# yizuo417/RollingDepth

Measured on AMD Instinct MI355X. Metric: depth frames/sec at 768px snip_len=3, 1-step denoise; 1/2/4/8 MI355X, higher is better.
Workload: dtype f16; 1 GPU; fast preset: 100-frame 768x768 video, dilations [1, 25] (cap_dilation=True), snippet_len 3, 1-step DDIM, aligner 2000 it, refine 0; SD2-shaped UNet+VAE random-init; preset=fast, frames=100, res=768, parallelism=snippet-dp1

## Files before the change

### include/rdmi.h

```cpp
#ifndef RDMI_H
#define RDMI_H

#include <stddef.h>

#ifdef __cplusplus
extern "C" {
#endif

#define RDMI_OK 0
#define RDMI_E_ARG 1001
#define RDMI_E_ALIGN 1002
#define RDMI_E_UNSUPPORTED 1003

#define RDMI_F16 0
#define RDMI_F32 1
#define RDMI_U8 2
#define RDMI_F32_X3 3
#define RDMI_F32_X6 4

#define RDMI_RESIZE_NEAREST 0
#define RDMI_RESIZE_BILINEAR 1
#define RDMI_RESIZE_BICUBIC 2

#define RDMI_EPI_NONE 0
// ... 105 lines not shown
  float* workspace;
  int start_step[8];
} rdmi_aligner_args;
long rdmi_aligner_workspace(const rdmi_aligner_args* a);
int rdmi_aligner_optimize(const rdmi_aligner_args* a, void* stream);
int rdmi_aligner_prepare(const void* x, int x_f32, int n, int w, int H, int W, int border,
                         int factor, const float* shift, float* out, void* stream);
int rdmi_aligner_merge(int n_dil, const void* const* xf, int x_f32, const float* const* s,
                       const float* const* t, const int* n, const int* stride, const int* w, int seq_len,
                       long HW, const float* shift, float* out, void* stream);
int rdmi_aligner_merge_strided(int n_dil, const void* const* xf, int x_f32, const float* const* s,
                               const float* const* t, const int* n, const int* stride, const int* start_step,
                               const int* w, int seq_len, long HW, const float* shift, float* out, void* stream);

int rdmi_aligner_merge_partial_window(int n_dil, const void* const* xf, int x_f32, const float* const* s,
                                      const float* const* t, const int* n, const int* stride, const int* k0,
                                      const int* nloc, const int* w, int f0, int nf, long HW, const float* shift,
                                      double* sum_out, void* stream);
int rdmi_aligner_merge_finish_pieces(int n_dil, const int* n, const int* stride, const int* w, int f0, int nf, long HW,
                                     int npieces, const int* piece_f0, const int* piece_nf, const double* recv,
                                     float* out, void* stream);
int rdmi_aligner_merge_partial_window_strided(int n_dil, const void* const* xf, int x_f32, const float* const* s,
                                              const float* const* t, const int* n, const int* stride,
                                              const int* start_step, const int* k0, const int* nloc, const int* w,
                                              int seq_len, int f0, int nf, long HW, const float* shift,
                                              double* sum_out, void* stream);
int rdmi_aligner_merge_finish_pieces_strided(int n_dil, const int* n, const int* stride, const int* start_step,
                                             const int* w, int seq_len, int f0, int nf, long HW, int npieces,
                                             const int* piece_f0, const int* piece_nf, const double* recv,
                                             float* out, void* stream);

int rdmi_attention_d512(const void* q, const void* k, const void* vt, void* o, int B, int Sq, int Sk, int Skp,
                        long q_ld, long k_ld, long vt_ld, long o_ld, long q_bs, long k_bs, long vt_bs, long o_bs,
                        float scale, int* flags, void* stream);

size_t rdmi_resize_workspace(int N, int C, int H, int W, int Ho, int Wo);
int rdmi_resize(const void* x, int x_dtype, long sn, long sc, long sy, long sx, int N, int C, int H, int W, int Ho,
                int Wo, int mode, int normalize, float* y, void* workspace, void* stream);

#ifdef __cplusplus
}
#endif
#endif
```

### rollingdepth_amd/_native.py

```python
from __future__ import annotations

import ctypes as C
import os

_LIB_PATH = os.environ.get("RDMI_LIB") or os.path.join(os.path.dirname(os.path.abspath(__file__)), "_lib", "librdmi.so")

vp = C.c_void_p
i32 = C.c_int
i64 = C.c_long
f32 = C.c_float


class GemmArgs(C.Structure):
    _fields_ = [
        ("A", vp), ("lda", i64), ("strideA", i64),
        ("W", vp), ("ldw", i64), ("strideW", i64),
        ("C", vp), ("ldc", i64), ("strideC", i64), ("c_f32", i32),
        ("bias", vp),
        ("residual", vp), ("ldr", i64), ("strideR", i64),
        ("rowbias", vp), ("rows_per_group", i32), ("rowbias_ld", i64),
        ("alpha", f32),
        ("M", i32), ("N", i32), ("K", i32), ("batch", i32),
        ("epilogue", i32),
        ("gn_part", vp), ("gn_ld", i64),
# ... 31 lines not shown
    ]


_SIGS = {
    "rdmi_last_error": (C.c_char_p, []),
    "rdmi_version": (i32, []),
    "rdmi_gemm": (i32, [C.POINTER(GemmArgs), vp]),
    "rdmi_conv2d": (i32, [C.POINTER(ConvArgs), vp]),
    "rdmi_conv2d_in_gn_supported": (i32, [C.POINTER(ConvArgs)]),
    "rdmi_groupnorm_workspace": (i64, [i32, i32]),
    "rdmi_groupnorm_stats": (i32, [vp, i32, i32, i64, i32, i32, f32, vp, vp, vp]),
    "rdmi_groupnorm_stats_partials": (i32, [vp, i64, i32, i64, i32, i32, f32, vp, vp]),
    "rdmi_groupnorm_apply": (i32, [vp, vp, i32, i32, i64, i32, i32, vp, vp, vp, i32, vp]),
    "rdmi_conv3x3_to1_gn_workspace": (i64, [i32, i32, i32]),
    "rdmi_conv3x3_to1_gn": (i32, [vp, i32, i32, i32, i32, i32, i32, vp, vp, vp, i32, vp, f32, vp, i32, vp, vp]),
    "rdmi_layernorm": (i32, [vp, vp, i32, i64, i32, vp, vp, f32, vp]),
    "rdmi_attention_fwd": (i32, [vp, vp, vp, vp, i32, i32, i32, i32, i32, i64, i64, i64, i64, i64, i64, i64, i64,
                                 f32, i32, vp]),
    "rdmi_attention_smallkv": (i32, [vp, vp, vp, vp, i32, i32, i32, i32, i32, i64, i64, i64, i64, i64, f32, i32, vp]),
    "rdmi_cross_attn_pair": (i32, [vp, vp, i64, i32, i32, vp, vp, f32, vp, vp, vp, vp]),
    "rdmi_softmax_rows": (i32, [vp, vp, i64, i64, i64, f32, i32, vp]),
    "rdmi_nchw_to_nhwc": (i32, [vp, i32, vp, i32, i32, i32, i32, i32, i32, f32, i64, i64, vp]),
    "rdmi_nhwc_to_nchw_f32": (i32, [vp, i32, i64, vp, i32, i32, i32, i32, f32, f32, vp]),
    "rdmi_concat_channels": (i32, [vp, i32, vp, i32, vp, i64, i32, vp]),
    "rdmi_resize_nearest": (i32, [vp, i32, i32, i32, i32, vp, i32, i32, i32, vp]),
    "rdmi_transpose": (i32, [vp, vp, i32, i64, i64, i64, i64, i32, vp]),
    "rdmi_gather_unet_input": (i32, [vp, i64, vp, i64, i32, vp, i32, i64, vp, i32, vp]),
    "rdmi_ddim_combine": (i32, [vp, i64, vp, i64, vp, i64, i64, i32, i32, f32, f32, f32, i64, i32, vp]),
    "rdmi_snippet_average": (i32, [vp, i32, i32, i32, i32, i64, i32, i32, vp, i32, vp]),
    "rdmi_snippet_accumulate": (i32, [vp, i32, i32, i32, i32, i32, i32, i64, i32, i32, vp, vp]),
    "rdmi_snippet_finish": (i32, [vp, i32, i32, i32, i32, i64, i32, i32, vp, i32, vp]),
    "rdmi_colorize": (i32, [vp, i32, i64, vp, vp, i32, vp, vp, vp]),
    "rdmi_resize_workspace": (C.c_size_t, [i32, i32, i32, i32, i32, i32]),
    "rdmi_attention_d512": (i32, [vp, vp, vp, vp, i32, i32, i32, i32] + [i64] * 8 + [C.c_float, vp, vp]),
    "rdmi_resize": (i32, [vp, i32, i64, i64, i64, i64, i32, i32, i32, i32, i32, i32, i32, i32, vp, vp, vp]),
    "rdmi_minmax": (i32, [vp, i32, i64, vp, vp, vp]),
    "rdmi_renormalize_f32": (i32, [vp, i64, vp, vp]),
    "rdmi_aligner_workspace": (i64, [C.POINTER(AlignerArgs)]),
    "rdmi_aligner_optimize": (i32, [C.POINTER(AlignerArgs), vp]),
    "rdmi_aligner_prepare": (i32, [vp, i32, i32, i32, i32, i32, i32, i32, vp, vp, vp]),
    "rdmi_aligner_merge": (i32, [i32, C.POINTER(vp), i32, C.POINTER(vp), C.POINTER(vp), C.POINTER(i32),
                                 C.POINTER(i32), C.POINTER(i32), i32, i64, vp, vp, vp]),
    "rdmi_aligner_merge_strided": (i32, [i32, C.POINTER(vp), i32, C.POINTER(vp), C.POINTER(vp), C.POINTER(i32),
                                         C.POINTER(i32), C.POINTER(i32), C.POINTER(i32), i32, i64, vp, vp, vp]),
    "rdmi_groupnorm_affine": (i32, [vp, vp, vp, i32, i32, i32, vp, vp]),
    "rdmi_aligner_merge_partial_window": (i32, [i32, C.POINTER(vp), i32, C.POINTER(vp), C.POINTER(vp),
                                                C.POINTER(i32), C.POINTER(i32), C.POINTER(i32), C.POINTER(i32),
                                                C.POINTER(i32), i32, i32, i64, vp, vp, vp]),
    "rdmi_aligner_merge_finish_pieces": (i32, [i32, C.POINTER(i32), C.POINTER(i32), C.POINTER(i32), i32, i32, i64,
                                               i32, C.POINTER(i32), C.POINTER(i32), vp, vp, vp]),
    "rdmi_aligner_merge_partial_window_strided": (i32, [i32, C.POINTER(vp), i32, C.POINTER(vp), C.POINTER(vp),
                                                        C.POINTER(i32), C.POINTER(i32), C.POINTER(i32),
                                                        C.POINTER(i32), C.POINTER(i32), C.POINTER(i32), i32, i32, i32,
                                                        i64, vp, vp, vp]),
    "rdmi_aligner_merge_finish_pieces_strided": (i32, [i32, C.POINTER(i32), C.POINTER(i32), C.POINTER(i32),
                                                       C.POINTER(i32), i32, i32, i32, i64, i32, C.POINTER(i32),
                                                       C.POINTER(i32), vp, vp, vp]),
}

RDMI_F16, RDMI_F32, RDMI_U8, RDMI_F32_X3, RDMI_F32_X6 = 0, 1, 2, 3, 4
RDMI_RESIZE_NEAREST, RDMI_RESIZE_BILINEAR, RDMI_RESIZE_BICUBIC = 0, 1, 2

EXPORTED = tuple(_SIGS)


def _load():
    if not os.path.exists(_LIB_PATH):
# ... 23 lines not shown
```

### rollingdepth_amd/csrc/attention_d512.hip

```cpp
#include "common.h"

namespace {

constexpr int D5 = 512;
constexpr int NW5 = 8;
constexpr int QB5 = 16 * NW5;
constexpr int KT5 = 32;
constexpr int KTILE = KT5 * D5;
constexpr int STAGE = 2 * KTILE;
constexpr int PPW = 32 / NW5;

__device__ __forceinline__ int kswz(int k) { return (k & 3) | (((k >> 3) & 3) << 2); }
__device__ __forceinline__ int vswz(int d) { return ((d >> 3) & 1) * 3; }

struct Attn512P {
  const f16* q; const f16* k; const f16* vt; f16* o;
  int Sq, Sk, Skp;
  long q_ld, k_ld, vt_ld, o_ld, q_bs, k_bs, vt_bs, o_bs;
  float c;
  int* flags;
};

__global__ __launch_bounds__(64 * NW5, 1) void attn_fwd_d512(Attn512P p) {
  __shared__ __attribute__((aligned(16))) f16 lds5[2 * STAGE];
// ... 102 lines not shown
#pragma unroll
          for (int db = 0; db < 32; ++db) o[db] *= alpha;
        }
        mt = mnew;
      }
      rs = 0.f;
#pragma unroll
      for (int e = 0; e < 8; ++e) {
        pv[e] = __builtin_amdgcn_exp2f(fmaf(s[e >> 2][e & 3], p.c, -mt));
        rs += pv[e];
      }
      rs += __shfl_xor(rs, 16, 64);
      rs += __shfl_xor(rs, 32, 64);
    }
    l += rs;
    f16x8 pf;
#pragma unroll
    for (int e = 0; e < 8; ++e) pf[e] = (f16)pv[e];
#pragma unroll
    for (int db = 0; db < 32; ++db) {
      const f16x8 vf = *(const f16x8*)LDS_PTR(f16, (uintptr_t)(st + vaddr + db * 1024));
      o[db] = __builtin_amdgcn_mfma_f32_16x16x32_f16(vf, pf, o[db], 0, 0, 0);
    }
  }
  if (q < p.Sq) {
    const float inv = 1.f / l;
    f16* O = p.o + (long)b * p.o_bs + (long)q * p.o_ld;
#pragma unroll
    for (int db = 0; db < 32; ++db) {
      f16x4 w;
#pragma unroll
      for (int r = 0; r < 4; ++r) w[r] = (f16)(o[db][r] * inv);
      *(f16x4*)(O + 16 * db + 4 * hq) = w;
    }
  }
}


__device__ __forceinline__ int kswz32(int k) { return k & 15; }
__device__ __forceinline__ int vswz32(int d) { return (d >> 2) & 3; }

template <int N>
__device__ __forceinline__ void w4_sched() {
#pragma unroll
  for (int i = 0; i < N; ++i) {
    __builtin_amdgcn_sched_group_barrier(0x100, 1, 0);
    __builtin_amdgcn_sched_group_barrier(0x008, 1, 0);
  }
}

__global__ __launch_bounds__(256, 1) void attn_fwd_d512_w4(Attn512P p) {
  __shared__ __attribute__((aligned(16))) f16 lds5[2 * STAGE];
  const int tid = threadIdx.x;
  const int lane = tid & 63;
  const int wid = tid >> 6;
  const int hh = lane >> 5;
  const int j32 = lane & 31;
  const int qblk = blockIdx.x, b = blockIdx.y;
  const int q = qblk * 128 + wid * 32 + j32;

  const f16* Q = p.q + (long)b * p.q_bs;
  const __amdgpu_buffer_rsrc_t rk = __builtin_amdgcn_make_buffer_rsrc(
      (void*)(p.k + (long)b * p.k_bs), (short)0, (int)(((long)(p.Sk - 1) * p.k_ld + D5) * 2), 0x00020000);
  const __amdgpu_buffer_rsrc_t rv = __builtin_amdgcn_make_buffer_rsrc(
      (void*)(p.vt + (long)b * p.vt_bs), (short)0, (int)(((long)(D5 - 1) * p.vt_ld + p.Skp) * 2), 0x00020000);

// ... 83 lines not shown
#pragma unroll
    for (int db = 0; db < 16; ++db)
#pragma unroll
      for (int s2 = 0; s2 < 2; ++s2) {
        const f16x8 vf = *(const f16x8*)LDS_PTR(f16, (uintptr_t)(st + vaddr[s2] + db * 2048));
        o[db] = __builtin_amdgcn_mfma_f32_32x32x16_f16(vf, pf[s2], o[db], 0, 0, 0);
      }
    w4_sched<32>();
  }
  int* badw = (int*)lds5;
  __syncthreads();
  if (lane == 0) badw[wid] = bad;
  __syncthreads();
  if (tid == 0) p.flags[b * gridDim.x + qblk] = badw[0] | badw[1] | badw[2] | badw[3];
  if (q < p.Sq && !bad) {
    const float inv = 1.f / l;
    f16* O = p.o + (long)b * p.o_bs + (long)q * p.o_ld;
#pragma unroll
    for (int db = 0; db < 16; ++db)
#pragma unroll
      for (int jx = 0; jx < 4; ++jx) {
        f16x4 w;
#pragma unroll
        for (int r = 0; r < 4; ++r) w[r] = (f16)(o[db][4 * jx + r] * inv);
        *(f16x4*)(O + 32 * db + 8 * jx + 4 * hh) = w;
      }
  }
}

}

extern "C" int rdmi_attention_d512(const void* q, const void* k, const void* vt, void* o, int B, int Sq, int Sk, int Skp,
                                   long q_ld, long k_ld, long vt_ld, long o_ld, long q_bs, long k_bs, long vt_bs,
                                   long o_bs, float scale, int* flags, void* stream) {
  RDMI_REQUIRE(q && k && vt && o, RDMI_E_ARG, "attention_d512: null pointer");
  RDMI_REQUIRE(B > 0 && Sq > 0 && Sk > 0 && Skp >= Sk && Skp % 32 == 0 && vt_ld >= Skp, RDMI_E_ARG,
               "attention_d512: bad sizes (Skp %% 32 == 0, Skp >= Sk, vt_ld >= Skp)");
  RDMI_REQUIRE(q_ld % 8 == 0 && k_ld % 8 == 0 && vt_ld % 8 == 0 && o_ld % 4 == 0 &&
                   (((uintptr_t)q | (uintptr_t)k | (uintptr_t)vt) & 15) == 0 && ((uintptr_t)o & 7) == 0,
               RDMI_E_ALIGN, "attention_d512: strides / pointers not aligned");
  RDMI_REQUIRE((long)(Sk - 1) * k_ld + D5 < (1L << 30) && (long)(D5 - 1) * vt_ld + Skp < (1L << 30), RDMI_E_ARG,
               "attention_d512: K / Vᵀ exceed the 2 GiB buffer range");
  Attn512P p{(const f16*)q, (const f16*)k, (const f16*)vt, (f16*)o, Sq, Sk, Skp, q_ld, k_ld, vt_ld, o_ld,
             q_bs, k_bs, vt_bs, o_bs, scale * 1.4426950408889634f, flags};
  const dim3 grid(rdmi::div_up(Sq, QB5), B);
  if (flags) {
    hipLaunchKernelGGL(attn_fwd_d512_w4, grid, dim3(256), 0, (hipStream_t)stream, p);
    if (int e = rdmi::check_launch("attention_d512 (32-query pass)")) return e;
  }
  hipLaunchKernelGGL(attn_fwd_d512, grid, dim3(64 * NW5), 0, (hipStream_t)stream, p);
  return rdmi::check_launch("attention_d512");
}
```

### rollingdepth_amd/kernels.py

```python
from __future__ import annotations

import ctypes as C
import math
import os
from typing import Optional, Sequence, Tuple

import torch

from . import _native as _N
from ._native import check, lib

F16 = torch.float16
F32 = torch.float32


def _stream() -> int:
    return torch.cuda.current_stream().cuda_stream


_PROF = None


def profile_start():
    global _PROF
# ... 615 lines not shown
    if out.numel() != rows * p_ld or not out.is_contiguous() or p_ld < cols:
        raise ValueError("softmax_rows: out must be a contiguous [..., >= cols] tensor")
    check(lib.rdmi_softmax_rows(s.data_ptr(), out.data_ptr(), rows, cols, p_ld, scale, _dtype_code(out), _stream()),
          "rdmi_softmax_rows")
    return out


def attention_1head(q: torch.Tensor, k: torch.Tensor, v: torch.Tensor, scale: float) -> torch.Tensor:
    B, Sq, D = q.shape
    Sk = k.shape[1]
    if D == 512 and q.dtype == F16 and os.environ.get("RDMI_VAE_FLASH", "1") != "0":
        return attention_d512(q, k, v, scale)
    s = gemm(q, k, D, out_f32=True)
    Sp = (Sk + 7) // 8 * 8
    p = softmax_rows(s, scale, out=torch.empty((B, Sq, Sp), dtype=q.dtype, device=q.device))
    del s
    vt = torch.zeros((B, D, Sp), dtype=q.dtype, device=q.device) if Sp != Sk else None
    vt = transpose(v, out=vt)
    return gemm(p, vt, Sp)


def attention_d512(q: torch.Tensor, k: torch.Tensor, v: torch.Tensor, scale: float) -> torch.Tensor:
    B, Sq, D = q.shape
    Sk = k.shape[1]
    if D != 512 or q.dtype != F16 or k.dtype != F16 or v.dtype != F16:
        raise ValueError("attention_d512: f16 q / k / v with head dim 512")
    Skp = (Sk + 31) // 32 * 32
    vt = torch.zeros((B, D, Skp), dtype=F16, device=q.device) if Skp != Sk else None
    vt = transpose(v, out=vt)
    o = torch.empty((B, Sq, D), dtype=F16, device=q.device)
    flags = None
    if os.environ.get("RDMI_D512_W4", "0") == "1":
        flags = torch.empty((B * ((Sq + 127) // 128),), dtype=torch.int32, device=q.device)
    with _Timed("attention_d512", 4.0 * B * Sq * Sk * D, f"attn512 B={B} S={Sq}", 2 * B * D * (2 * Sq + 2 * Sk)):
        check(lib.rdmi_attention_d512(q.data_ptr(), k.data_ptr(), vt.data_ptr(), o.data_ptr(), B, Sq, Sk, Skp,
                                      q.stride(1), k.stride(1), vt.stride(1), o.stride(1), q.stride(0), k.stride(0),
                                      vt.stride(0), o.stride(0), float(scale),
                                      flags.data_ptr() if flags is not None else None, _stream()),
              "rdmi_attention_d512")
    return o


def transpose(src: torch.Tensor, out: Optional[torch.Tensor] = None) -> torch.Tensor:
    _need_act(src, "transpose.src")
    B, R, Cc = src.shape
    out = torch.empty((B, Cc, R), dtype=src.dtype, device=src.device) if out is None else out
    for t, rows, nm in ((src, R, "src"), (out, Cc, "out")):
        if t.stride(2) != 1 or (B > 1 and t.stride(0) != rows * t.stride(1)):
            raise ValueError(f"transpose: {nm} strides {t.stride()} (unit column stride, batch stride = rows · row "
                             f"stride expected)")
    check(lib.rdmi_transpose(src.data_ptr(), out.data_ptr(), B, R, Cc, src.stride(1), out.stride(1), _dtype_code(src),
                             _stream()), "rdmi_transpose")
    return out


def nchw_to_nhwc(x: torch.Tensor, cpad: int, scale: float = 1.0, dtype=F16) -> torch.Tensor:
    if not x.is_cuda or x.dtype not in (F16, F32):
        raise TypeError("nchw_to_nhwc: device f16/f32 tensor expected")
    B, Cc, H, W = x.shape
    if x.stride(3) != 1 or x.stride(2) != W:
        x = x.contiguous()
    out = torch.empty((B, H, W, cpad), dtype=dtype, device=x.device)
    check(lib.rdmi_nchw_to_nhwc(x.data_ptr(), int(x.dtype == F32), out.data_ptr(), _dtype_code(out), B, Cc, H, W, cpad,
                                scale, x.stride(0), x.stride(1), _stream()), "rdmi_nchw_to_nhwc")
    return out


def nhwc_to_nchw_f32(x: torch.Tensor, c: int, scale: float = 1.0, shift: float = 0.0) -> torch.Tensor:
    _need_act(x, "nhwc_to_nchw.x")
    B, H, W, Cl = x.shape
# ... 285 lines not shown
```

### rollingdepth_amd/csrc/conv_occ2.hip

```cpp
#include "gemm_kernels.h"

namespace rdmi_gk {

template <int MODE>
static void occ2_mode_launch(bool gn, bool pipe, dim3 g, hipStream_t s, const GemmP& p) {
  if (gn && pipe)
    hipLaunchKernelGGL((conv_halo_occ2_kernel<MODE, true, true>), g, dim3(256), 0, s, p);
  else if (gn)
    hipLaunchKernelGGL((conv_halo_occ2_kernel<MODE, true, false>), g, dim3(256), 0, s, p);
  else if (pipe)
    hipLaunchKernelGGL((conv_halo_occ2_kernel<MODE, false, true>), g, dim3(256), 0, s, p);
  else
    hipLaunchKernelGGL((conv_halo_occ2_kernel<MODE, false, false>), g, dim3(256), 0, s, p);
}

void launch_conv_occ2(int mode, bool gn, bool pipe, dim3 g, hipStream_t s, const GemmP& p) {
  if (mode == 3) {
    if (pipe)
      hipLaunchKernelGGL((conv_halo_occ2_kernel<3, false, true>), g, dim3(256), 0, s, p);
    else
      hipLaunchKernelGGL((conv_halo_occ2_kernel<3, false, false>), g, dim3(256), 0, s, p);
  } else if (mode == 2)
    occ2_mode_launch<2>(gn, pipe, g, s, p);
  else
    occ2_mode_launch<1>(gn, pipe, g, s, p);
}

void launch_conv_h32(bool gn, dim3 g, hipStream_t s, const GemmP& p) {
  if (gn)
    hipLaunchKernelGGL((conv_halo32_kernel<true>), g, dim3(256), 0, s, p);
  else
    hipLaunchKernelGGL((conv_halo32_kernel<false>), g, dim3(256), 0, s, p);
}

void launch_gemm_occ2(int bn, dim3 g, hipStream_t s, const GemmP& p) {
  if (bn == 160 && !p.geglu)
    hipLaunchKernelGGL((gemm_occ2_kernel<0, 160>), g, dim3(256), 0, s, p);
  else
    hipLaunchKernelGGL((gemm_occ2_kernel<0, 128>), g, dim3(256), 0, s, p);
}

}
```

### rollingdepth_amd/csrc/gemm.hip

```cpp
#include "gemm_kernels.h"

#include <stdlib.h>

namespace {

using namespace rdmi_gk;


int occ2_mode() {
  const char* e = getenv("RDMI_GEMM_OCC2");
  return e ? atoi(e) : 1;
}

int pp_mode() {
  const char* e = getenv("RDMI_GEMM_PP");
  return e ? atoi(e) : 1;
}

double tile_cost(long tiles, int bm, int bn, double eff) {
  return (double)((tiles + 255) / 256) * bm * bn / eff;
}

template <int MODE, int WM, int RN>
void launch_pp(const GemmP& p, int batch, hipStream_t s) {
// ... 206 lines not shown
    const char* xp = getenv("RDMI_XFORM_PRIO");
    p.xprio = !(xp && xp[0] == '0');
    const char* ep = getenv("RDMI_EPI_PRIO");
    p.eprio = ep && ep[0] == '1';
    const char* cp = getenv("RDMI_CPERM");
    p.cperm = (!cp || cp[0] != '0') && p.vec && ((uintptr_t)p.C & 15) == 0 && p.ldc % 8 == 0 &&
              (!p.R || (((uintptr_t)p.R & 15) == 0 && p.ldr % 8 == 0));
    p.gmr = a->in_mean_rstd; p.ggam = a->in_gamma; p.gbet = a->in_beta; p.gG = a->in_groups; p.gsilu = a->in_silu;
    p.gaff = a->in_mean_rstd ? a->in_affine : nullptr;
    RDMI_REQUIRE(!p.gaff || ((uintptr_t)p.gaff & 15) == 0, RDMI_E_ALIGN, "conv2d: in_affine not 16-byte aligned");
    hipStream_t st = (hipStream_t)stream;
    const unsigned patches = (unsigned)((a->Ho / 16) * (a->Wo / 16) * a->B);
    const bool gn = p.gmr != nullptr;
    if (a->upsample && a->w_up2 && !gn && a->Ho % 32 == 0 && a->Wo % 32 == 0 && al16(a->w_up2)) {
      p.Wt = (const f16*)a->w_up2; p.ldw = 7L * a->Cin; p.K = p.Kvalid = 7 * a->Cin;
      p.w_bytes = (unsigned)(4L * a->Cout * p.ldw * 2);
      launch_conv_occ2(3, false, p.conv_pipe != 0, dim3((a->Cout + 127) / 128, patches, 1), st, p);
    } else if (a->Cout % 256 == 0 && !p.gaff && !(hmode == 3 && (!gn || a->Cin <= 256))) {
      dim3 g(a->Cout / 256, patches, 1);
      const bool ph2 = hmode != 1 || gn;
      if (a->upsample) {
        launch_conv_halo(2, ph2 ? 2 : 4, 4, ph2 && gn, g, st, p);
      } else {
        launch_conv_halo(1, ph2 ? 2 : 4, 4, ph2 && gn, g, st, p);
      }
    } else if (a->Cout == 128 && !p.gaff && (hmode == 4 || (gn && a->Cin > 256))) {
      dim3 g(1, patches, 1);
      launch_conv_halo(a->upsample ? 2 : 1, 1, 2, gn, g, st, p);
    } else if (h32_ok(a, p, gn)) {
      dim3 g(a->Cout / 128, (unsigned)((a->Ho / 8) * (a->Wo / 32) * a->B), 1);
      launch_conv_h32(gn, g, st, p);
    } else {
      dim3 g((a->Cout + 127) / 128, patches, 1);
      launch_conv_occ2(a->upsample ? 2 : 1, gn, p.conv_pipe != 0, g, st, p);
    }
    return rdmi::check_launch("conv2d halo");
  }
  if (dense && conv1x1_ok(p) && launch_conv1x1(p, a->Cin, a->Cout, (hipStream_t)stream))
    return rdmi::check_launch("conv2d 1x1");
  return launch(p, 1, (hipStream_t)stream, false, dense ? 0 : (a->upsample ? 2 : 1));
}
```

### rollingdepth_amd/csrc/gemm_kernels.h

```cpp
#pragma once
#include "common.h"

#include <utility>

namespace rdmi_gk {

constexpr int BK = 64;

struct GemmP {
  const f16* A; long lda, sA;
  const f16* Wt; long ldw, sW;
  void* C; long ldc, sC; int c_f32;
  const float* bias;
  const f16* R; long ldr, sR;
  const float* rowbias; int rpg; long rb_ld;
  float alpha;
  int M, N, K, Kvalid;
  int geglu, silu, vec;
  unsigned a_bytes, w_bytes;
  int IH, IW, Cin, Ho, Wo, kh, kw, stride, pt, pl, up, cin_vecs;
  int cmaj;
  float* gnp; long gn_ld;
  int group_m;
  const float* gmr; const float* ggam; const float* gbet; int gG, gsilu;
// ... 1122 lines not shown
      asm volatile("" ::: "memory");
      __builtin_amdgcn_s_barrier();
      asm volatile("" ::: "memory");
      seg(5);
    }
  }
  if (grp == 0) __builtin_amdgcn_s_barrier();
  wait_vmcnt<0>();
  seg(5);

  store_tile<RM, RN, 64, true>(p, acc, PatchRows{b, p.Ho, p.Wo, y0, x0, wm * RM, fr}, n0 + wn * 64, 0, fr, fq, p.cperm);
  if constexpr (STAMP) {
    wait_vmcnt<0>();
    seg(6);
    st_acc[7] = st_prev - st_start;
    if (lane == 0) {
      unsigned long long* o = p.stamps + (((long)blockIdx.y * gridDim.x + blockIdx.x) * 8 + wid) * 8;
      for (int i = 0; i < 8; ++i) o[i] = st_acc[i];
    }
  }
}

template <int RN, int PD, int NS, int BPRE, int ST>
__device__ __forceinline__ void occ2_sched_one() {
  constexpr int nr = (ST == BPRE ? RN : 0) + (ST + PD < NS ? 1 : 0);
  if constexpr (nr > 0) __builtin_amdgcn_sched_group_barrier(0x100, nr, 0);
  __builtin_amdgcn_sched_group_barrier(0x008, RN, 0);
}
template <int RN, int PD, int NS, int BPRE, int... S>
__device__ __forceinline__ void occ2_sched(std::integer_sequence<int, S...>) {
  (occ2_sched_one<RN, PD, NS, BPRE, S>(), ...);
}

template <int MODE, bool GN, bool PIPE, int STAMP = 0>
__global__ __launch_bounds__(256, 2) void conv_halo_occ2_kernel(GemmP p) {
  unsigned long long st_acc[6] = {}, st_prev = 0, st_start = 0;
  auto seg = [&](int i) __attribute__((always_inline)) {
    if constexpr (STAMP) {
      const unsigned long long t = gk_stamp();
      st_acc[i] += t - st_prev;
      st_prev = t;
    }
  };
  if constexpr (STAMP) st_start = st_prev = gk_stamp();
  constexpr int BN = 128, BKP = 64, RM = 8, RN = 4;
  constexpr int HWD = 18, HPIX = HWD * HWD;
  constexpr int HPC = 41;
  constexpr int HPW = 11;
  constexpr int HALO = HPC * 8 * BKP;
  constexpr int BSLOT = BN * BKP;
  constexpr int NB = 4;
  constexpr int GNT = GN ? 256 : 0;
  constexpr int PREF = 4 * 2 * 64 * 2;
  __shared__ __attribute__((aligned(16))) f16 lds[HALO + 2 * BSLOT + 4 * GNT + PREF];
  float* const gnt = (float*)(lds + HALO + 2 * BSLOT);

  const int tid = threadIdx.x;
  const int lane = tid & 63;
  const int wid = tid >> 6;
  const int wm = wid >> 1, wn = wid & 1;
  const int wids = __builtin_amdgcn_readfirstlane(wid);
  const int nbx = gridDim.x;
  int mt_, nt_;
  if (p.group_m < 0 && nbx > 1 && 8 % nbx == 0 && gridDim.y % (8 / nbx) == 0) {
    const int bid = blockIdx.y * nbx + blockIdx.x, xcd = bid & 7;
    nt_ = xcd % nbx;
    mt_ = (bid >> 3) * (8 / nbx) + xcd / nbx;
  } else {
    const int logical = xcd_remap(blockIdx.y * nbx + blockIdx.x, nbx * gridDim.y);
    tile_mn(logical, nbx, gridDim.y, p.group_m, mt_, nt_);
  }
  const int n0 = nt_ * BN;
  constexpr int NT = MODE == 3 ? 7 : 9;
  const int pxn = p.Wo >> (MODE == 3 ? 5 : 4), pyn = p.Ho >> (MODE == 3 ? 5 : 4);
  const int px = mt_ % pxn;
  const int py = (mt_ / pxn) % pyn;
  const int phs = MODE == 3 ? (mt_ / (pxn * pyn)) & 3 : 0;
  const int b = mt_ / (pxn * pyn * (MODE == 3 ? 4 : 1));
  const int pa = phs >> 1, pc = phs & 1;
  const int y0 = py * 16, x0 = px * 16;
  const __amdgpu_buffer_rsrc_t ra_ =
      __builtin_amdgcn_make_buffer_rsrc((void*)p.A, (short)0, (int)p.a_bytes, 0x00020000);
  const __amdgpu_buffer_rsrc_t rw_ =
      __builtin_amdgcn_make_buffer_rsrc((void*)p.Wt, (short)0, (int)p.w_bytes, 0x00020000);

  const int lrow = lane >> 3;
  const int chunk = (lane & 7) ^ lrow;
  const int Hl = p.IH << (MODE == 2 ? 1 : 0), Wl = p.IW << (MODE == 2 ? 1 : 0);
  unsigned hvo[HPW];
#pragma unroll
  for (int e = 0; e < HPW; ++e) {
    const int hp = (wid + 4 * e) * 8 + lrow;
    const int hr = hp / HWD, hc = hp - hr * HWD;
    const int yy = y0 - 1 + pa + hr, xx = x0 - 1 + pc + hc;
    const bool ok = hp < HPIX && (unsigned)yy < (unsigned)Hl && (unsigned)xx < (unsigned)Wl;
    const int sy = MODE == 2 ? yy >> 1 : yy, sx = MODE == 2 ? xx >> 1 : xx;
    hvo[e] = ok ? (unsigned)(((b * p.IH + sy) * p.IW + sx) * p.Cin + chunk * 8) * 2u : OOB;
  }
  unsigned pvo[2];
#pragma unroll
  for (int j = 0; j < 2; ++j) {
    const int idx = j * 64 + lane, e = idx >> 3;
    const int hp = (wid + 4 * e) * 8 + (idx & 7);
    const int hr = hp / HWD, hc = hp - hr * HWD;
    const int yy = y0 - 1 + pa + hr, xx = x0 - 1 + pc + hc;
    const bool ok = e < HPW && wid + 4 * e < HPC && hp < HPIX && (unsigned)yy < (unsigned)Hl && (unsigned)xx < (unsigned)Wl;
    const int sy = MODE == 2 ? yy >> 1 : yy, sx = MODE == 2 ? xx >> 1 : xx;
    pvo[j] = ok ? (unsigned)(((b * p.IH + sy) * p.IW + sx) * p.Cin) * 2u : OOB;
  }
  auto prefetchHalo = [&](int cb) {
    f16* lp = lds + HALO + 2 * BSLOT + 4 * GNT + wids * 256;
#pragma unroll
    for (int j = 0; j < 2; ++j)
      __builtin_amdgcn_raw_ptr_buffer_load_lds(ra_, (__attribute__((address_space(3))) void*)(lp + j * 128), 4,
                                               pvo[j], cb * 128, 0, 0);
  };
  unsigned bvo[NB];
#pragma unroll
  for (int e = 0; e < NB; ++e) {
    const int rt = (wid + 4 * e) * 8 + lrow;
    const int n = n0 + (p.cperm ? (rt & ~63) + perm64(rt & 63) : rt);
    bvo[e] = n < p.N ? (unsigned)((phs * p.N + n) * (int)p.ldw + chunk * 8) * 2u : OOB;
  }
  const int ncb = p.Cin >> 6;
  auto hv = [&](int e) { return wids + 4 * e < HPC; };
  auto issueHalo = [&](int cb) {
#pragma unroll
    for (int e = 0; e < HPW; ++e)
      if (hv(e)) {
        f16* lh = lds + (wids + 4 * e) * 8 * BKP;
        dma16s(ra_, hvo[e], cb * 128, lh);
      }
  };
  auto issueB = [&](int u) {
    f16* lb = lds + HALO + (u & 1) * BSLOT;
#pragma unroll
    for (int e = 0; e < NB; ++e) dma16s(rw_, bvo[e], u * BKP * 2, lb + (wids + 4 * e) * 8 * BKP);
  };
  f32x4 aff[4];
  auto loadAff = [&](int cb) {
    if (p.gaff) {
      const float* ta = p.gaff + ((long)b * ncb + cb) * 128 + chunk * 8;
      aff[0] = *(const f32x4*)ta;
      aff[1] = *(const f32x4*)(ta + 4);
      aff[2] = *(const f32x4*)(ta + 64);
      aff[3] = *(const f32x4*)(ta + 68);
    }
  };
  auto xformHalo = [&](int cb) {
    if (!p.gaff) {
      const float* ts = gnt + cb * 64 + chunk * 8;
      aff[0] = *(const f32x4*)ts;
      aff[1] = *(const f32x4*)(ts + 4);
      aff[2] = *(const f32x4*)(ts + GNT);
      aff[3] = *(const f32x4*)(ts + GNT + 4);
    }
    const float sc[8] = {aff[0][0], aff[0][1], aff[0][2], aff[0][3], aff[1][0], aff[1][1], aff[1][2], aff[1][3]};
    const float sh[8] = {aff[2][0], aff[2][1], aff[2][2], aff[2][3], aff[3][0], aff[3][1], aff[3][2], aff[3][3]};
    unsigned wn[4];
    *(f16x8*)wn = *(const f16x8*)(lds + wid * 8 * BKP + lane * 8);
#pragma unroll
    for (int e = 0; e < HPW; ++e)
      if (hv(e)) {
// ... 27 lines not shown
  if (GN && !p.gaff) {
    const int c = tid;
    float mean = 0.f, rstd = 0.f, gm = 0.f, bt = 0.f;
    if (c < p.Cin) {
      const int g = c / (p.Cin / p.gG);
      mean = p.gmr[2 * (b * p.gG + g)];
      rstd = p.gmr[2 * (b * p.gG + g) + 1];
      gm = p.ggam[c];
      bt = p.gbet[c];
    }
    const float sc = rstd * gm;
    gnt[c] = sc;
    gnt[GNT + c] = bt - mean * sc;
  }
  wait_vmcnt<0>();
  asm volatile("s_waitcnt lgkmcnt(0)" ::: "memory");
  __builtin_amdgcn_s_barrier();
  if constexpr (GN) {
    if (p.xprio) __builtin_amdgcn_s_setprio(2);
    xformHalo(0);
    if (p.xprio) __builtin_amdgcn_s_setprio(0);
    __builtin_amdgcn_s_barrier();
  }
  asm volatile("" ::: "memory");

  const int wms = __builtin_amdgcn_readfirstlane(wm);
  const bool live = n0 + (wids & 1) * 64 < p.N;
  seg(0);
  for (int u = 0; u < nk; ++u) {
    const int cb = u / NT;
    const int tap = u - cb * NT;
    const int t4 = tap < 4 ? tap : tap - 4 + (tap - 4 >= phs ? 1 : 0);
    const int dy = MODE == 3 ? t4 >> 1 : (tap * 11) >> 5, dx = MODE == 3 ? t4 & 1 : tap - 3 * dy;
    const bool pf = p.halo_pref && cb + 1 < ncb && NT > 2;
    if (u > 0) seg(2);
    if (u > 0) {
      if (tap == 0) {
        asm volatile("s_waitcnt lgkmcnt(0)" ::: "memory");
        __builtin_amdgcn_s_barrier();
        asm volatile("" ::: "memory");
        issueHalo(cb);
        if constexpr (GN) loadAff(cb);
        wait_vmcnt<0>();
        if constexpr (GN) {
          if (p.xprio) __builtin_amdgcn_s_setprio(2);
          xformHalo(cb);
          if (p.xprio) __builtin_amdgcn_s_setprio(0);
        }
      } else {
        if (pf && tap == 2)
          wait_vmcnt<2>();
        else
          wait_vmcnt<0>();
        asm volatile("s_waitcnt lgkmcnt(0)" ::: "memory");
      }
      asm volatile("" ::: "memory");
      __builtin_amdgcn_s_barrier();
      asm volatile("" ::: "memory");
      if (tap == 0) seg(3); else seg(1);
    }
    if (u + 1 < nk) issueB(u + 1);
    if (pf && tap == 1) prefetchHalo(cb + 1);
    const f16* lb = lds + HALO + (u & 1) * BSLOT + (wn * 64) * BKP;
    const int xb = fr + dx + 2 * dy;
    const unsigned abase = (unsigned)(((wms * RM + dy) * HWD + dx + fr) * BKP * 2);
    unsigned aoff[4];
#pragma unroll
    for (int r = 0; r < 4; ++r) aoff[r] = abase + (unsigned)((fq ^ ((xb + 2 * r) & 7)) << 4);
    auto readA = [&](int kh, int i) {
      const unsigned a = kh ? (aoff[i & 3] ^ 64u) : aoff[i & 3];
      return *(const f16x8*)((const char*)lds + a + i * HWD * BKP * 2);
    };
    if (live) {
      if constexpr (PIPE) {
        constexpr int NS = 2 * RM, PD = 2, BPRE = RM - 3;
        f16x8 bfr[2][RN], ar[PD + 1];
#pragma unroll
        for (int j = 0; j < RN; ++j) bfr[0][j] = *(const f16x8*)(lb + j * 16 * BKP + off0);
#pragma unroll
        for (int q = 0; q < PD; ++q) ar[q] = readA(q / RM, q % RM);
#pragma unroll
        for (int st = 0; st < NS; ++st) {
          if (st == BPRE) {
#pragma unroll
            for (int j = 0; j < RN; ++j) bfr[1][j] = *(const f16x8*)(lb + j * 16 * BKP + off1);
          }
          if (st + PD < NS) ar[(st + PD) % (PD + 1)] = readA((st + PD) / RM, (st + PD) % RM);
          const int kh = st / RM, i = st % RM;
#pragma unroll
          for (int j = 0; j < RN; ++j)
            acc[i][j] = __builtin_amdgcn_mfma_f32_16x16x32_f16(bfr[kh][j], ar[st % (PD + 1)], acc[i][j], 0, 0, 0);
        }
        __builtin_amdgcn_sched_group_barrier(0x100, RN + PD, 0);
        occ2_sched<RN, PD, NS, BPRE>(std::make_integer_sequence<int, NS>{});
      } else {
        f16x8 af[2][RM], bf[2][RN];
#pragma unroll
        for (int kh = 0; kh < 2; ++kh) {
          const int off = kh ? off1 : off0;
#pragma unroll
          for (int j = 0; j < RN; ++j) bf[kh][j] = *(const f16x8*)(lb + j * 16 * BKP + off);
#pragma unroll
          for (int i = 0; i < RM; ++i) af[kh][i] = readA(kh, i);
        }
// ... 484 lines not shown
```

Before: 23.73 depth frames/s.

## Add software-pipelined split attention kernel for head-dim 512 overlapping QK and PV

Adds a new d512 attention kernel that software-pipelines across K tiles. Each tile computes QK^T and softmax for tile t while doing the PV MFMAs for tile t-1, with P and rescale factors exchanged through LDS and sched_group_barrier hints to interleave the two. Rescaling of the output accumulator is lazy: it is skipped unless the row max grows enough. It is enabled by default through an env flag, and trades extra LDS and synchronisation for better MFMA utilisation in the VAE mid-block attention.

Measured after the change: 23.85 depth frames/s, median of 6. No clear change (+0.5%).

```diff
diff --git a/include/rdmi.h b/include/rdmi.h
--- a/include/rdmi.h
+++ b/include/rdmi.h
@@ -161,7 +161,7 @@
 
 int rdmi_attention_d512(const void* q, const void* k, const void* vt, void* o, int B, int Sq, int Sk, int Skp,
                         long q_ld, long k_ld, long vt_ld, long o_ld, long q_bs, long k_bs, long vt_bs, long o_bs,
-                        float scale, int* flags, void* stream);
+                        float scale, int split, int* flags, void* stream);
 
 size_t rdmi_resize_workspace(int N, int C, int H, int W, int Ho, int Wo);
 int rdmi_resize(const void* x, int x_dtype, long sn, long sc, long sy, long sx, int N, int C, int H, int W, int Ho,
diff --git a/rollingdepth_amd/_native.py b/rollingdepth_amd/_native.py
--- a/rollingdepth_amd/_native.py
+++ b/rollingdepth_amd/_native.py
@@ -87,7 +87,7 @@
     "rdmi_snippet_finish": (i32, [vp, i32, i32, i32, i32, i64, i32, i32, vp, i32, vp]),
     "rdmi_colorize": (i32, [vp, i32, i64, vp, vp, i32, vp, vp, vp]),
     "rdmi_resize_workspace": (C.c_size_t, [i32, i32, i32, i32, i32, i32]),
-    "rdmi_attention_d512": (i32, [vp, vp, vp, vp, i32, i32, i32, i32] + [i64] * 8 + [C.c_float, vp, vp]),
+    "rdmi_attention_d512": (i32, [vp, vp, vp, vp, i32, i32, i32, i32] + [i64] * 8 + [C.c_float, i32, vp, vp]),
     "rdmi_resize": (i32, [vp, i32, i64, i64, i64, i64, i32, i32, i32, i32, i32, i32, i32, i32, vp, vp, vp]),
     "rdmi_minmax": (i32, [vp, i32, i64, vp, vp, vp]),
     "rdmi_renormalize_f32": (i32, [vp, i64, vp, vp]),
diff --git a/rollingdepth_amd/csrc/attention_d512.hip b/rollingdepth_amd/csrc/attention_d512.hip
--- a/rollingdepth_amd/csrc/attention_d512.hip
+++ b/rollingdepth_amd/csrc/attention_d512.hip
@@ -158,6 +158,234 @@
 #pragma unroll
       for (int r = 0; r < 4; ++r) w[r] = (f16)(o[db][r] * inv);
       *(f16x4*)(O + 16 * db + 4 * hq) = w;
+    }
+  }
+}
+
+
+constexpr int PBUF = 8 * 64 * 8;
+constexpr int TAB5 = 2 * STAGE + 2 * PBUF;
+constexpr int TAB_FLAG = 2 * 128 * 4;
+constexpr int TAB_INV = TAB_FLAG + 2 * 8 * 4;
+
+template <int MASK, int N>
+__device__ __forceinline__ void sgb() { __builtin_amdgcn_sched_group_barrier(MASK, N, 0); }
+
+__global__ __launch_bounds__(64 * NW5, 1) void attn_fwd_d512_split(Attn512P p) {
+  __shared__ __attribute__((aligned(16))) f16 lds5[TAB5 + 1024];
+  const int tid = threadIdx.x;
+  const int lane = tid & 63;
+  const int wid = __builtin_amdgcn_readfirstlane(tid >> 6);
+  const int hq = lane >> 4;
+  const int j16 = lane & 15;
+  const int qblk = blockIdx.x, b = blockIdx.y;
+  const int q = qblk * QB5 + wid * 16 + j16;
+
+  const f16* Q = p.q + (long)b * p.q_bs;
+  const __amdgpu_buffer_rsrc_t rk = __builtin_amdgcn_make_buffer_rsrc(
+      (void*)(p.k + (long)b * p.k_bs), (short)0, (int)(((long)(p.Sk - 1) * p.k_ld + D5) * 2), 0x00020000);
+  const __amdgpu_buffer_rsrc_t rv = __builtin_amdgcn_make_buffer_rsrc(
+      (void*)(p.vt + (long)b * p.vt_bs), (short)0, (int)(((long)(D5 - 1) * p.vt_ld + p.Skp) * 2), 0x00020000);
+
+  f16x8 qf[16];
+#pragma unroll
+  for (int ks = 0; ks < 16; ++ks) {
+    f16x8 z = {};
+    qf[ks] = q < p.Sq ? *(const f16x8*)(Q + (long)q * p.q_ld + ks * 32 + hq * 8) : z;
+  }
+
+  const unsigned kvo = (unsigned)((lane ^ kswz(PPW * wid)) << 4);
+  const unsigned vvo = (unsigned)(((lane >> 2) * p.vt_ld + (((lane & 3) ^ vswz(lane >> 2)) << 3)) * 2);
+  auto issue_k = [&](int t) {
+    f16* st = lds5 + (t & 1) * STAGE;
+    unsigned x = kvo;
+    asm volatile("" : "+v"(x));
+#pragma unroll
+    for (int e = 0; e < PPW; ++e)
+      __builtin_amdgcn_raw_ptr_buffer_load_lds(rk, (__attribute__((address_space(3))) void*)(st + (PPW * wid + e) * 512),
+                                               16, (x ^ (e << 4)) + (unsigned)((PPW * wid + e) * (int)p.k_ld * 2),
+                                               t * KT5 * (int)p.k_ld * 2, 0, 0);
+  };
+  auto issue_v = [&](int t) {
+    f16* st = lds5 + (t & 1) * STAGE;
+    unsigned x = vvo;
+    asm volatile("" : "+v"(x));
+#pragma unroll
+    for (int e = 0; e < PPW; ++e)
+      __builtin_amdgcn_raw_ptr_buffer_load_lds(rv, (__attribute__((address_space(3))) void*)(st + KTILE + (PPW * wid + e) * 512),
+                                               16, x + (unsigned)(16 * (PPW * wid + e) * (int)p.vt_ld * 2),
+                                               t * KT5 * 2, 0, 0);
+  };
+
+  const unsigned base0 = (unsigned)(uintptr_t)LDS_PTR(f16, lds5);
+  unsigned kcur[4], vaddr;
+  {
+    const int kap = 8 * (j16 >> 2) + (j16 & 3);
+#pragma unroll
+    for (int b4 = 0; b4 < 4; ++b4) kcur[b4] = base0 + (unsigned)(kap * 1024 + (((4 * b4 + hq) ^ kswz(kap)) << 4));
+  }
+  vaddr = (unsigned)(KTILE * 2 + wid * 4096 + j16 * 64 + ((hq ^ vswz(j16)) << 4));
+  const unsigned pbase = base0 + 2 * STAGE * 2 + lane * 16;
+  const unsigned tab = base0 + TAB5 * 2;
+  const unsigned tabq = tab + j16 * 4;
+
+  f32x4 o[8][4];
+#pragma unroll
+  for (int g = 0; g < 8; ++g)
+#pragma unroll
+    for (int dbl = 0; dbl < 4; ++dbl) o[g][dbl] = f32x4{0.f, 0.f, 0.f, 0.f};
+  float mt = 0.f, l = 0.f;
+
+  auto tile = [&](const int t, auto has_pv, auto has_qk) {
+    constexpr bool PV = decltype(has_pv)::value, QK = decltype(has_qk)::value;
+    const unsigned stv = base0 + (unsigned)(((t & 1) ^ 1) * STAGE * 2);
+    const int pb = (t & 1) ^ 1;
+    const unsigned pin = pbase + pb * 8192, ain = tabq + pb * 512;
+    int fl = 0;
+    if constexpr (PV) fl = *(const int*)LDS_PTR(int, (uintptr_t)(tab + TAB_FLAG + pb * 32 + (lane & 7) * 4));
+    f32x4 s[2] = {};
+    if constexpr (QK) {
+#pragma unroll
+      for (int ks = 0; ks < 16; ++ks)
+#pragma unroll
+        for (int kb = 0; kb < 2; ++kb) {
+          const f16x8 kf = *(const f16x8*)LDS_PTR(f16, (uintptr_t)(kcur[ks & 3] + (kb * 4096 + (ks >> 2) * 256)));
+          s[kb] = __builtin_amdgcn_mfma_f32_16x16x32_f16(kf, qf[ks], s[kb], 0, 0, 0);
+        }
+#pragma unroll
+      for (int b4 = 0; b4 < 4; ++b4) kcur[b4] += (t & 1) ? (unsigned)(-STAGE * 2) : (unsigned)(STAGE * 2);
+      const int lim = p.Sk - t * KT5 - 8 * hq;
+#pragma unroll
+      for (int kb = 0; kb < 2; ++kb)
+#pragma unroll
+        for (int r = 0; r < 4; ++r) s[kb][r] = 4 * kb + r >= lim ? -INFINITY : s[kb][r];
+    }
+    f16x8 vf[4] = {};
+    if constexpr (PV) {
+#pragma unroll
+      for (int dbl = 0; dbl < 4; ++dbl) vf[dbl] = *(const f16x8*)LDS_PTR(f16, (uintptr_t)(stv + vaddr + dbl * 1024));
+      if constexpr (QK) {
+        sgb<0x100, 5>();
+#pragma unroll
+        for (int i = 0; i < 32; ++i) {
+          sgb<0x008, 1>();
+          sgb<0x100, 1>();
+        }
+      }
+      const unsigned mask = (unsigned)__ballot(fl != 0) & 0xffu;
+      if (mask) {
+#pragma unroll
+        for (int g = 0; g < 8; ++g)
+          if ((mask >> g) & 1) {
+            const float alpha = *(const float*)LDS_PTR(float, (uintptr_t)(ain + g * 64));
+#pragma unroll
+            for (int dbl = 0; dbl < 4; ++dbl) o[g][dbl] *= alpha;
+          }
+      }
+    }
+    float pv[8];
+    float rs = 0.f;
+#pragma unroll
+    for (int g = 0; g < 8; ++g) {
+      if constexpr (PV) {
+        const f16x8 pg = *(const f16x8*)LDS_PTR(f16, (uintptr_t)(pin + g * 1024));
+#pragma unroll
+        for (int dbl = 0; dbl < 4; ++dbl)
+          o[g][dbl] = __builtin_amdgcn_mfma_f32_16x16x32_f16(vf[dbl], pg, o[g][dbl], 0, 0, 0);
+      }
+      if constexpr (QK) {
+        pv[g] = __builtin_amdgcn_exp2f(fmaf(s[g >> 2][g & 3], p.c, -mt));
+        rs += pv[g];
+      }
+    }
+    if constexpr (PV && QK) {
+      sgb<0x100, 2>();
+#pragma unroll
+      for (int g = 0; g < 6; ++g) {
+        sgb<0x008, 4>();
+        sgb<0x100, 1>();
+      }
+      sgb<0x008, 8>();
+    }
+    if constexpr (QK) {
+      rs += __shfl_xor(rs, 16, 64);
+      rs += __shfl_xor(rs, 32, 64);
+      bool hit = false;
+      float apub = 1.f;
+      if (t == 0 || __any(!(rs <= 32768.f))) {
+        float mx = -INFINITY;
+#pragma unroll
+        for (int e = 0; e < 8; ++e) mx = fmaxf(mx, s[e >> 2][e & 3] * p.c);
+        mx = fmaxf(mx, __shfl_xor(mx, 16, 64));
+        mx = fmaxf(mx, __shfl_xor(mx, 32, 64));
+        const float mnew = t == 0 ? mx : fmaxf(mt, mx);
+        if (t == 0 || mnew > mt) {
+          const float alpha = t == 0 ? 0.f : __builtin_amdgcn_exp2f(mt - mnew);
+          l *= alpha;
+          if (t != 0) {
+            hit = true;
+            apub = alpha;
+          }
+          mt = mnew;
+        }
+        rs = 0.f;
+#pragma unroll
+        for (int e = 0; e < 8; ++e) {
+          pv[e] = __builtin_amdgcn_exp2f(fmaf(s[e >> 2][e & 3], p.c, -mt));
+          rs += pv[e];
+        }
+        rs += __shfl_xor(rs, 16, 64);
+        rs += __shfl_xor(rs, 32, 64);
+      }
+      l += rs;
+      f16x8 pf;
+#pragma unroll
+      for (int e = 0; e < 8; ++e) pf[e] = (f16)pv[e];
+      *(f16x8*)LDS_PTR(f16, (uintptr_t)(pbase + ((t & 1) * 8 + wid) * 1024)) = pf;
+      const int anyhit = __any(hit);
+      if (anyhit && lane < 16)
+        *(float*)LDS_PTR(float, (uintptr_t)(tab + (t & 1) * 512 + (wid * 16 + lane) * 4)) = apub;
+      if (lane == 0) *(int*)LDS_PTR(int, (uintptr_t)(tab + TAB_FLAG + (t & 1) * 32 + wid * 4)) = anyhit;
+    }
+  };
+  auto sync = [&]() {
+    __builtin_amdgcn_s_waitcnt(0x7 << 4);
+    asm volatile("" ::: "memory");
+    __builtin_amdgcn_s_barrier();
+    asm volatile("" ::: "memory");
+  };
+
+  const int nt = p.Skp / KT5;
+  issue_k(0);
+  sync();
+  if (1 < nt) issue_k(1);
+  issue_v(0);
+  tile(0, std::false_type{}, std::true_type{});
+  for (int t = 1; t < nt; ++t) {
+    sync();
+    if (t + 1 < nt) issue_k(t + 1);
+    issue_v(t);
+    tile(t, std::true_type{}, std::true_type{});
+  }
+  if (lane < 16) *(float*)LDS_PTR(float, (uintptr_t)(tab + TAB_INV + (wid * 16 + lane) * 4)) = 1.f / l;
+  sync();
+  tile(nt, std::true_type{}, std::false_type{});
+
+  int le = lane;
+  asm volatile("" : "+v"(le));
+  f16* O = p.o + (long)b * p.o_bs + 64 * wid + 4 * (le >> 4);
+#pragma unroll
+  for (int g = 0; g < 8; ++g) {
+    const int qg = qblk * QB5 + g * 16 + (le & 15);
+    const float inv = *(const float*)LDS_PTR(float, (uintptr_t)(tabq + TAB_INV + g * 64));
+    if (qg < p.Sq) {
+#pragma unroll
+      for (int dbl = 0; dbl < 4; ++dbl) {
+        f16x4 w;
+#pragma unroll
+        for (int r = 0; r < 4; ++r) w[r] = (f16)(o[g][dbl][r] * inv);
+        *(f16x4*)(O + (long)qg * p.o_ld + 16 * dbl) = w;
+      }
     }
   }
 }
@@ -307,7 +535,7 @@
 
 extern "C" int rdmi_attention_d512(const void* q, const void* k, const void* vt, void* o, int B, int Sq, int Sk, int Skp,
                                    long q_ld, long k_ld, long vt_ld, long o_ld, long q_bs, long k_bs, long vt_bs,
-                                   long o_bs, float scale, int* flags, void* stream) {
+                                   long o_bs, float scale, int split, int* flags, void* stream) {
   RDMI_REQUIRE(q && k && vt && o, RDMI_E_ARG, "attention_d512: null pointer");
   RDMI_REQUIRE(B > 0 && Sq > 0 && Sk > 0 && Skp >= Sk && Skp % 32 == 0 && vt_ld >= Skp, RDMI_E_ARG,
                "attention_d512: bad sizes (Skp %% 32 == 0, Skp >= Sk, vt_ld >= Skp)");
@@ -322,6 +550,9 @@
   if (flags) {
     hipLaunchKernelGGL(attn_fwd_d512_w4, grid, dim3(256), 0, (hipStream_t)stream, p);
     if (int e = rdmi::check_launch("attention_d512 (32-query pass)")) return e;
+  } else if (split) {
+    hipLaunchKernelGGL(attn_fwd_d512_split, grid, dim3(64 * NW5), 0, (hipStream_t)stream, p);
+    return rdmi::check_launch("attention_d512 (split)");
   }
   hipLaunchKernelGGL(attn_fwd_d512, grid, dim3(64 * NW5), 0, (hipStream_t)stream, p);
   return rdmi::check_launch("attention_d512");
diff --git a/rollingdepth_amd/kernels.py b/rollingdepth_amd/kernels.py
--- a/rollingdepth_amd/kernels.py
+++ b/rollingdepth_amd/kernels.py
@@ -671,10 +671,11 @@
     flags = None
     if os.environ.get("RDMI_D512_W4", "0") == "1":
         flags = torch.empty((B * ((Sq + 127) // 128),), dtype=torch.int32, device=q.device)
+    split = 0 if os.environ.get("RDMI_D512_SPLIT", "1") == "0" else 1
     with _Timed("attention_d512", 4.0 * B * Sq * Sk * D, f"attn512 B={B} S={Sq}", 2 * B * D * (2 * Sq + 2 * Sk)):
         check(lib.rdmi_attention_d512(q.data_ptr(), k.data_ptr(), vt.data_ptr(), o.data_ptr(), B, Sq, Sk, Skp,
                                       q.stride(1), k.stride(1), vt.stride(1), o.stride(1), q.stride(0), k.stride(0),
-                                      vt.stride(0), o.stride(0), float(scale),
+                                      vt.stride(0), o.stride(0), float(scale), split,
                                       flags.data_ptr() if flags is not None else None, _stream()),
               "rdmi_attention_d512")
     return o
```

## Load source-resolution halo for non-GN upsample convs with double-buffered prefetch

Applied to the files above, without the earlier changes.

Adds a MODE 4 variant of the occ2 halo conv for upsample convs without GroupNorm. It stages a 10x10 source-resolution halo instead of the 18x18 upsampled one and maps output pixels to source pixels when reading A fragments, using a new swizzle. The smaller halo is double-buffered and the next channel block is prefetched during the current one, which removes the per-block halo barrier and stall. This cuts global reads and LDS footprint, at the cost of more complex addressing, possible LDS bank conflicts from duplicated reads, and new waitcnt accounting that must be exactly right.

New measurement: 22.94 depth frames/s before, 23.05 depth frames/s after (median of 6 runs). No clear change (+0.5%).

```diff
diff --git a/rollingdepth_amd/csrc/conv_occ2.hip b/rollingdepth_amd/csrc/conv_occ2.hip
--- a/rollingdepth_amd/csrc/conv_occ2.hip
+++ b/rollingdepth_amd/csrc/conv_occ2.hip
@@ -20,6 +20,11 @@
       hipLaunchKernelGGL((conv_halo_occ2_kernel<3, false, true>), g, dim3(256), 0, s, p);
     else
       hipLaunchKernelGGL((conv_halo_occ2_kernel<3, false, false>), g, dim3(256), 0, s, p);
+  } else if (mode == 4) {
+    if (pipe)
+      hipLaunchKernelGGL((conv_halo_occ2_kernel<4, false, true>), g, dim3(256), 0, s, p);
+    else
+      hipLaunchKernelGGL((conv_halo_occ2_kernel<4, false, false>), g, dim3(256), 0, s, p);
   } else if (mode == 2)
     occ2_mode_launch<2>(gn, pipe, g, s, p);
   else
diff --git a/rollingdepth_amd/csrc/gemm.hip b/rollingdepth_amd/csrc/gemm.hip
--- a/rollingdepth_amd/csrc/gemm.hip
+++ b/rollingdepth_amd/csrc/gemm.hip
@@ -262,7 +262,9 @@
       launch_conv_h32(gn, g, st, p);
     } else {
       dim3 g((a->Cout + 127) / 128, patches, 1);
-      launch_conv_occ2(a->upsample ? 2 : 1, gn, p.conv_pipe != 0, g, st, p);
+      const char* sh = getenv("RDMI_UP_SRC_HALO");
+      const bool src = a->upsample && !gn && !(sh && sh[0] == '0');
+      launch_conv_occ2(a->upsample ? (src ? 4 : 2) : 1, gn, p.conv_pipe != 0, g, st, p);
     }
     return rdmi::check_launch("conv2d halo");
   }
diff --git a/rollingdepth_amd/csrc/gemm_kernels.h b/rollingdepth_amd/csrc/gemm_kernels.h
--- a/rollingdepth_amd/csrc/gemm_kernels.h
+++ b/rollingdepth_amd/csrc/gemm_kernels.h
@@ -1178,6 +1178,8 @@
   (occ2_sched_one<RN, PD, NS, BPRE, S>(), ...);
 }
 
+__device__ __forceinline__ int src_swz(int pair) { return ((pair & 3) | ((pair >> 1) & 2)) << 1; }
+
 template <int MODE, bool GN, bool PIPE, int STAMP = 0>
 __global__ __launch_bounds__(256, 2) void conv_halo_occ2_kernel(GemmP p) {
   unsigned long long st_acc[6] = {}, st_prev = 0, st_start = 0;
@@ -1190,10 +1192,14 @@
   };
   if constexpr (STAMP) st_start = st_prev = gk_stamp();
   constexpr int BN = 128, BKP = 64, RM = 8, RN = 4;
-  constexpr int HWD = 18, HPIX = HWD * HWD;
-  constexpr int HPC = 41;
-  constexpr int HPW = 11;
-  constexpr int HALO = HPC * 8 * BKP;
+  constexpr bool SRC = MODE == 4;
+  constexpr bool UP = MODE == 2 || SRC;
+  static_assert(!(SRC && GN), "the source-resolution halo has no in-place GroupNorm transform");
+  constexpr int HWD = SRC ? 10 : 18, HPIX = HWD * HWD;
+  constexpr int HPC = SRC ? 13 : 41;
+  constexpr int HPW = SRC ? 4 : 11;
+  constexpr int HBUF = HPC * 8 * BKP;
+  constexpr int HALO = (SRC ? 2 : 1) * HBUF;
   constexpr int BSLOT = BN * BKP;
   constexpr int NB = 4;
   constexpr int GNT = GN ? 256 : 0;
@@ -1232,16 +1238,17 @@
 
   const int lrow = lane >> 3;
   const int chunk = (lane & 7) ^ lrow;
-  const int Hl = p.IH << (MODE == 2 ? 1 : 0), Wl = p.IW << (MODE == 2 ? 1 : 0);
+  const int Hl = p.IH << (UP && !SRC ? 1 : 0), Wl = p.IW << (UP && !SRC ? 1 : 0);
   unsigned hvo[HPW];
 #pragma unroll
   for (int e = 0; e < HPW; ++e) {
     const int hp = (wid + 4 * e) * 8 + lrow;
     const int hr = hp / HWD, hc = hp - hr * HWD;
-    const int yy = y0 - 1 + pa + hr, xx = x0 - 1 + pc + hc;
+    const int yy = (SRC ? y0 >> 1 : y0) - 1 + pa + hr, xx = (SRC ? x0 >> 1 : x0) - 1 + pc + hc;
     const bool ok = hp < HPIX && (unsigned)yy < (unsigned)Hl && (unsigned)xx < (unsigned)Wl;
     const int sy = MODE == 2 ? yy >> 1 : yy, sx = MODE == 2 ? xx >> 1 : xx;
-    hvo[e] = ok ? (unsigned)(((b * p.IH + sy) * p.IW + sx) * p.Cin + chunk * 8) * 2u : OOB;
+    const int hchunk = SRC ? (lane & 7) ^ src_swz(hc >> 1) : chunk;
+    hvo[e] = ok ? (unsigned)(((b * p.IH + sy) * p.IW + sx) * p.Cin + hchunk * 8) * 2u : OOB;
   }
   unsigned pvo[2];
 #pragma unroll
@@ -1274,7 +1281,7 @@
 #pragma unroll
     for (int e = 0; e < HPW; ++e)
       if (hv(e)) {
-        f16* lh = lds + (wids + 4 * e) * 8 * BKP;
+        f16* lh = lds + (SRC ? (cb & 1) * HBUF : 0) + (wids + 4 * e) * 8 * BKP;
         dma16s(ra_, hvo[e], cb * 128, lh);
       }
   };
@@ -1368,10 +1375,11 @@
     const int tap = u - cb * NT;
     const int t4 = tap < 4 ? tap : tap - 4 + (tap - 4 >= phs ? 1 : 0);
     const int dy = MODE == 3 ? t4 >> 1 : (tap * 11) >> 5, dx = MODE == 3 ? t4 & 1 : tap - 3 * dy;
-    const bool pf = p.halo_pref && cb + 1 < ncb && NT > 2;
+    const bool pf = !SRC && p.halo_pref && cb + 1 < ncb && NT > 2;
+    const bool nh = SRC && cb + 1 < ncb;
     if (u > 0) seg(2);
     if (u > 0) {
-      if (tap == 0) {
+      if (!SRC && tap == 0) {
         asm volatile("s_waitcnt lgkmcnt(0)" ::: "memory");
         __builtin_amdgcn_s_barrier();
         asm volatile("" ::: "memory");
@@ -1386,6 +1394,10 @@
       } else {
         if (pf && tap == 2)
           wait_vmcnt<2>();
+        else if (nh && tap == 1 && wids == 0)
+          wait_vmcnt<4>();
+        else if (nh && tap == 1)
+          wait_vmcnt<3>();
         else
           wait_vmcnt<0>();
         asm volatile("s_waitcnt lgkmcnt(0)" ::: "memory");
@@ -1393,19 +1405,27 @@
       asm volatile("" ::: "memory");
       __builtin_amdgcn_s_barrier();
       asm volatile("" ::: "memory");
-      if (tap == 0) seg(3); else seg(1);
+      if (!SRC && tap == 0) seg(3); else seg(1);
     }
     if (u + 1 < nk) issueB(u + 1);
+    if (nh && tap == 0) issueHalo(cb + 1);
     if (pf && tap == 1) prefetchHalo(cb + 1);
     const f16* lb = lds + HALO + (u & 1) * BSLOT + (wn * 64) * BKP;
     const int xb = fr + dx + 2 * dy;
-    const unsigned abase = (unsigned)(((wms * RM + dy) * HWD + dx + fr) * BKP * 2);
+    const int r0 = wms * RM + dy + 1, sc = (dx + fr + 1) >> 1;
+    const unsigned abase = SRC ? (unsigned)((cb & 1) * HBUF * 2 + ((r0 >> 1) * HWD + sc) * BKP * 2)
+                               : (unsigned)(((wms * RM + dy) * HWD + dx + fr) * BKP * 2);
     unsigned aoff[4];
-#pragma unroll
-    for (int r = 0; r < 4; ++r) aoff[r] = abase + (unsigned)((fq ^ ((xb + 2 * r) & 7)) << 4);
+    if constexpr (SRC) {
+      aoff[0] = aoff[2] = abase + (unsigned)((fq ^ src_swz(sc >> 1)) << 4);
+      aoff[1] = aoff[3] = aoff[0] + (unsigned)((r0 & 1) * HWD * BKP * 2);
+    } else {
+#pragma unroll
+      for (int r = 0; r < 4; ++r) aoff[r] = abase + (unsigned)((fq ^ ((xb + 2 * r) & 7)) << 4);
+    }
     auto readA = [&](int kh, int i) {
       const unsigned a = kh ? (aoff[i & 3] ^ 64u) : aoff[i & 3];
-      return *(const f16x8*)((const char*)lds + a + i * HWD * BKP * 2);
+      return *(const f16x8*)((const char*)lds + a + (SRC ? i >> 1 : i) * HWD * BKP * 2);
     };
     if (live) {
       if constexpr (PIPE) {
```
